# rwickman/ArbitraryStyleTransfer

Hardware: AMD Instinct MI355X
Metric: stylised images/sec at 512x512 bs=8, 1->8 MI355X; encoder MFMA %-of-peak (higher is better)
Workload: dtype f32

## Files before the change

arbitrarystyletransfer_amd/_lib.py:

```python
from __future__ import annotations

import ctypes
import os

import torch

_HERE = os.path.dirname(os.path.abspath(__file__))
LIB_PATH = os.environ.get("AST_HIP_LIB") or os.path.join(_HERE, "libast_hip.so")

_c_float_p = ctypes.c_void_p
_i = ctypes.c_int
_ll = ctypes.c_longlong
_p = ctypes.c_void_p
_f = ctypes.c_float
_d = ctypes.c_double

SIGNATURES = {
    "ast_version": (ctypes.c_char_p, []),
    "ast_loss_acc_floats": (_i, []),
    "ast_conv3x3_packed_numel": (ctypes.c_size_t, [_i, _i]),
    "ast_conv3x3_pack_weights_f32": (_i, [_p, _p, _i, _i, _p]),
    "ast_conv3x3_pack_split_f32": (_i, [_p, _i, _i, _p]),
    "ast_conv3x3_fwd_f32": (_i, [_p, _p, _p, _p, _p, _p, _p, _p, _i, _i, _i, _i, _i, _i, _i, _p]),
    "ast_conv3x3_num_configs": (_i, []),
    "ast_conv3x3_fwd_f32_cfg": (_i, [_i, _p, _p, _i, _p, _p, _p, _p, _p, _p, _p, _i, _i, _i, _i, _i, _i, _i, _p]),
    "ast_channel_stats_f32": (_i, [_p, _p, _p, _ll, _ll, _i, ctypes.c_float, _p]),
    "ast_adain_f32": (_i, [_p, _p, _p, _i, _i, _i, _i, _i, _i, ctypes.c_double, _i, _p]),
    "ast_plane_normalize_f32": (_i, [_p, _p, _p, _p, _ll, _ll, _p]),
    "ast_adain_backward_f32": (_i, [_p, _p, _p, _p, _p, _i, _i, _i, _i, _i, _i, _d, _i, _p]),
    "ast_adain_stats_f32": (_i, [_p, _p, _p, _p, _i, _i, _i, _i, _i, _d, _i, _p]),
    "ast_conv3x3_pack_weights_ex_f32": (_i, [_p, _p, _i, _i, _i, _p, _p]),
    "ast_conv_act_backward_f32": (_i, [_p, _p, _p, _p, _p, _ll, _i, _i, _p]),
    "ast_relu_mask_f32": (_i, [_p, _p, _p, _ll, _p]),
    "ast_grad_pad_f32": (_i, [_p, _p, _p, _ll, _i, _i, _i, _p]),
    "ast_pad_up_adjoint_f32": (_i, [_p, _p, _ll, _i, _i, _i, _i, _p]),
    "ast_conv3x3_dgrad_f32": (_i, [_i, _p, _p, _p, _p, _p, _p, _i, _i, _i, _i, _i, _i, _p]),
    "ast_dgrad_finish_f32": (_i, [_p, _p, _p, _p, _p, _ll, _i, _i, _i, _p]),
    "ast_dgrad_reflect_border_workspace_floats": (_ll, [_i, _i, _i, _i, _i, _i]),
    "ast_dgrad_reflect_border_f32": (_i, [_p, _p, _p, _p, _p, _ll, _i, _i, _i, _i, _i, _i, _p]),
    "ast_conv3x3_wgrad_workspace_floats": (_ll, [_i, _i, _i, _i, _i, _i]),
# ... 167 lines not shown
```

arbitrarystyletransfer_amd/csrc/conv3x3_igemm.hip:

```cpp
#include <hip/hip_runtime.h>
#include <stdint.h>
#include "../../include/ast_hip.h"
#include "x3.h"
#include "cin3.h"

namespace {

typedef float f32x16 __attribute__((ext_vector_type(16)));
typedef float f32x4 __attribute__((ext_vector_type(4)));

constexpr int TW = 32;

struct ConvArgs {
  const float* x;
  const float* x2;
  int nsplit;
  const float* wp;
  const float* bias;
  float* y_pre;
  float* y_act;
  float* y_pool;
  const float* in_mean;
  const float* in_std;
  int N, Cin, Hin, Win, Cout, H, W;
// ... 996 lines not shown
        rec[196] = 0x57a3u;
      }
    }
#endif
  } else {
#if X3_STAGED_EPI
    __syncthreads();
    store_tiles_staged<RM, RN>(a, acc, n, x0, y0, wm * RM, n0, h, l32, lane,
                               reinterpret_cast<float*>(x3_smem) + wm * 32 * RM * 36);
#else
    store_tiles<RM, RN>(a, acc, n, x0, y0, wm * RM, n0, h, l32);
#endif
  }
  if constexpr (!PER) break;
  }
}

__device__ __forceinline__ void x3_lds_barrier() { asm volatile("s_waitcnt lgkmcnt(0)\n\ts_barrier" ::: "memory"); }
__device__ __forceinline__ const float* x3p_uniform(const float* p) {
  const uint64_t v = reinterpret_cast<uint64_t>(p);
  const uint32_t lo = __builtin_amdgcn_readfirstlane((uint32_t)v), hi = __builtin_amdgcn_readfirstlane((uint32_t)(v >> 32));
  return reinterpret_cast<const float*>(((uint64_t)hi << 32) | lo);
}
__device__ __forceinline__ const ConvArgs& x3p_args() {
  auto p = __builtin_amdgcn_kernarg_segment_ptr();
  asm volatile("" : "+s"(p));
  return *(const ConvArgs*)p;
}

template <int WM, int RM, int RN, int UP, int OCC>
// ... 793 lines not shown
  return (int)hipGetLastError();
}

template <int WM, int RM, int RN, int OCC = 1>
int launch_x3p(const ConvArgs& a, hipStream_t s, int up) {
  if (a.in_mean) return AST_E_UNSUPPORTED;
  if ((int64_t)a.Cin * a.Hin * a.Win * 4 >= ((int64_t)1 << 31)) return AST_E_UNSUPPORTED;
  return up == 2 ? launch_x3p_one<WM, RM, RN, 2, OCC>(a, s) : launch_x3p_one<WM, RM, RN, 1, OCC>(a, s);
}

template <int WM, int RM, int RN, int OCC = 1, bool M16 = false, bool PER = false>
int launch_x3(const ConvArgs& a, hipStream_t s, int up) {
  if (a.in_mean) return AST_E_UNSUPPORTED;
  if ((int64_t)a.Cin * a.Hin * a.Win * 4 >= ((int64_t)1 << 31)) return AST_E_UNSUPPORTED;
  return up == 2 ? launch_x3_one<WM, RM, RN, 2, OCC, M16, PER>(a, s) : launch_x3_one<WM, RM, RN, 1, OCC, M16, PER>(a, s);
}

struct CfgEntry {
  int (*fn)(const ConvArgs&, hipStream_t, int);
  int bn;
  int th;
  int rm;
  int max_cout;
};

const CfgEntry kConfigs[] = {
    {launch_cfg<4, 1, 2, 2, 8>, 64, 8, 2, 0},
    {launch_cfg<4, 1, 2, 2, 4>, 64, 8, 2, 0},
    {launch_cfg<2, 2, 4, 2, 4>, 128, 8, 4, 0},
    {launch_cfg<2, 2, 2, 2, 8>, 128, 4, 2, 0},
// ... 82 lines not shown

int ast_conv3x3_pack_weights_f32(const float* w, float* w_packed, int cout, int cin, void* stream) {
  if (!w || !w_packed) return AST_E_NULLPTR;
  if (cout <= 0 || cin <= 0) return AST_E_SHAPE;
  const int cout_pad = round_up(cout, kCoutAlign), cin_pad = round_up(cin, kCinAlign);
  const int64_t total = (int64_t)cin_pad * 9 * cout_pad;
  const int blocks = (int)std::min<int64_t>((total + 255) / 256, 4096);
  hipLaunchKernelGGL(pack_weights_kernel, dim3(blocks), dim3(256), 0, (hipStream_t)stream, w, w_packed, cout, cin,
                     cout_pad, cin_pad);
  const int e = (int)hipGetLastError();
  return e ? e : ast_conv3x3_pack_split_f32(w_packed, cout, cin, stream);
}

int ast_conv3x3_num_configs(void) { return kNumConfigs; }

#if X3_STAMP
int ast_dbg_x3_stamps(void* host, size_t bytes, int clear) {
  const size_t n = std::min(bytes, sizeof(x3_stamp_buf));
  if (clear) {
    void* d = nullptr;
    const hipError_t e = hipGetSymbolAddress(&d, HIP_SYMBOL(x3_stamp_buf));
    return e ? (int)e : (int)hipMemset(d, 0, sizeof(x3_stamp_buf));
  }
  return (int)hipMemcpyFromSymbol(host, HIP_SYMBOL(x3_stamp_buf), n, 0, hipMemcpyDeviceToHost);
}
#endif

int ast_conv3x3_fwd_f32_cfg(int cfg, const float* x, const float* x2, int n2, const float* w_packed,
                            const float* bias, float* y_pre, float* y_act, float* y_pool, const float* in_mean,
                            const float* in_std, int n, int cin, int h_in, int w_in, int cout, int upsample,
// ... 87 lines not shown
```

arbitrarystyletransfer_amd/csrc/torch_ops.cpp:

```cpp
#include <torch/library.h>
#include <ATen/ATen.h>
#include <c10/hip/HIPStream.h>
#include <c10/core/DeviceGuard.h>

#include <tuple>

#include "../../include/ast_hip.h"

namespace {

void* cur_stream(const at::Tensor& t) {
  return (void*)c10::hip::getCurrentHIPStream(t.device().index()).stream();
}

const char* err_name(int code) {
  switch (code) {
    case AST_E_NULLPTR: return "null pointer";
    case AST_E_SHAPE: return "bad shape";
    case AST_E_UNSUPPORTED: return "unsupported configuration";
    default: return "hipError_t";
  }
}

#define AST_CALL(what, expr)                                                                    \
// ... 43 lines not shown
  const c10::DeviceGuard guard(x.device());
  at::Tensor mean = at::empty({x.size(0), x.size(1), 1, 1}, x.options());
  at::Tensor std_ = at::empty_like(mean);
  AST_CALL("channel_stats", ast_channel_stats_f32(x.data_ptr<float>(), mean.data_ptr<float>(), std_.data_ptr<float>(),
                                                  x.size(0) * x.size(1), x.size(2) * x.size(3), unbiased ? 1 : 0,
                                                  (float)eps, cur_stream(x)));
  return {mean, std_};
}

std::tuple<at::Tensor, at::Tensor> channel_stats_meta(const at::Tensor& x, bool, double) {
  TORCH_CHECK(x.dim() == 4, "channel_stats expects NCHW, got ", x.sizes());
  at::Tensor mean = at::empty({x.size(0), x.size(1), 1, 1}, x.options());
  return {mean, at::empty_like(mean)};
}

at::Tensor conv3x3_pack(const at::Tensor& w_) {
  at::Tensor w = dev_f32(w_, "weight");
  TORCH_CHECK(w.dim() == 4 && w.size(2) == 3 && w.size(3) == 3, "conv3x3 weight must be [cout, cin, 3, 3], got ",
              w.sizes());
  const int cout = (int)w.size(0), cin = (int)w.size(1);
  const c10::DeviceGuard guard(w.device());
  at::Tensor out = at::empty({(int64_t)ast_conv3x3_packed_numel(cout, cin)}, w.options());
  AST_CALL("conv3x3_pack", ast_conv3x3_pack_weights_f32(w.data_ptr<float>(), out.data_ptr<float>(), cout, cin,
                                                        cur_stream(w)));
  return out;
}

at::Tensor conv3x3_pack_meta(const at::Tensor& w) {
  TORCH_CHECK(w.dim() == 4 && w.size(2) == 3 && w.size(3) == 3, "conv3x3 weight must be [cout, cin, 3, 3], got ",
              w.sizes());
  return at::empty({(int64_t)ast_conv3x3_packed_numel((int)w.size(0), (int)w.size(1))}, w.options());
}

struct ConvShape {
  int64_t n, cin, h_in, w_in, H, W;
};

ConvShape conv_shape(const at::Tensor& x, const at::Tensor& w_packed, int64_t cout, int64_t upsample,
                     int64_t pad_mode, bool want_pre, bool want_act, bool want_pool) {
  TORCH_CHECK(x.dim() == 4, "x must be NCHW, got ", x.sizes());
  TORCH_CHECK(upsample == 1 || upsample == 2, "upsample must be 1 or 2");
  TORCH_CHECK(pad_mode == 0 || pad_mode == 1, "pad_mode must be 0 (zeros) or 1 (reflect)");
  TORCH_CHECK(want_pre || want_act || want_pool, "conv3x3: no output requested");
  TORCH_CHECK(cout > 0, "cout must be positive");
  ConvShape s{x.size(0), x.size(1), x.size(2), x.size(3), x.size(2) * upsample, x.size(3) * upsample};
  TORCH_CHECK(w_packed.numel() == (int64_t)ast_conv3x3_packed_numel((int)cout, (int)s.cin),
              "packed weight does not match (cout, cin)");
  TORCH_CHECK(!want_pool || (s.H >= 2 && s.W >= 2), "max-pool needs H, W >= 2");
  return s;
}

std::tuple<at::Tensor, at::Tensor, at::Tensor> conv3x3_fwd(
    const at::Tensor& x_, const at::Tensor& w_packed_, const c10::optional<at::Tensor>& bias_, int64_t cout,
    int64_t upsample, int64_t pad_mode, const c10::optional<at::Tensor>& in_mean_,
    const c10::optional<at::Tensor>& in_std_, bool want_pre, bool want_act, bool want_pool, int64_t cfg) {
  at::Tensor x = dev_f32(x_, "x"), w_packed = dev_f32(w_packed_, "w_packed");
  same_device(x, w_packed, "w_packed");
  const ConvShape s = conv_shape(x, w_packed, cout, upsample, pad_mode, want_pre, want_act, want_pool);
  c10::optional<at::Tensor> bias, in_mean, in_std;
  if (bias_) {
    bias = dev_f32(*bias_, "bias");
// ... 1 lines not shown
    TORCH_CHECK(bias->numel() == cout, "bias size mismatch");
  }
  TORCH_CHECK(in_mean_.has_value() == in_std_.has_value(), "in_mean and in_std go together");
  if (in_mean_) {
    in_mean = dev_f32(*in_mean_, "in_mean");
    in_std = dev_f32(*in_std_, "in_std");
    same_device(x, *in_mean, "in_mean");
    same_device(x, *in_std, "in_std");
    TORCH_CHECK(in_mean->numel() == s.cin && in_std->numel() == s.cin, "normalisation stats must have cin entries");
  }
  const c10::DeviceGuard guard(x.device());
  auto mk = [&](bool want, int64_t h, int64_t w) {
    return want ? at::empty({s.n, cout, h, w}, x.options()) : at::empty({0}, x.options());
  };
  at::Tensor pre = mk(want_pre, s.H, s.W), act = mk(want_act, s.H, s.W), pool = mk(want_pool, s.H / 2, s.W / 2);
  AST_CALL("conv3x3", ast_conv3x3_fwd_f32_cfg(
                          (int)cfg, x.data_ptr<float>(), nullptr, 0, w_packed.data_ptr<float>(), fptr(bias),
                          want_pre ? pre.data_ptr<float>() : nullptr, want_act ? act.data_ptr<float>() : nullptr,
                          want_pool ? pool.data_ptr<float>() : nullptr, fptr(in_mean), fptr(in_std), (int)s.n,
                          (int)s.cin, (int)s.h_in, (int)s.w_in, (int)cout, (int)upsample, (int)pad_mode,
                          cur_stream(x)));
  return {pre, act, pool};
}

std::tuple<at::Tensor, at::Tensor, at::Tensor> conv3x3_fwd_meta(
    const at::Tensor& x, const at::Tensor& w_packed, const c10::optional<at::Tensor>&, int64_t cout,
    int64_t upsample, int64_t pad_mode, const c10::optional<at::Tensor>&, const c10::optional<at::Tensor>&,
    bool want_pre, bool want_act, bool want_pool, int64_t) {
  const ConvShape s = conv_shape(x, w_packed, cout, upsample, pad_mode, want_pre, want_act, want_pool);
  auto mk = [&](bool want, int64_t h, int64_t w) {
// ... 13 lines not shown
  AST_CALL("gram", ast_gram_f32(f.data_ptr<float>(), g.data_ptr<float>(), (int)b, (int)c, hw,
                                (float)(1.0 / (double)(c * hw)), ws.data_ptr<float>(), wsf, cur_stream(f)));
  return g;
}

at::Tensor gram_meta(const at::Tensor& f) {
  TORCH_CHECK(f.dim() == 4, "gram_matrix expects [B, C, H, W], got ", f.sizes());
  return at::empty({f.size(0), f.size(1), f.size(1)}, f.options());
}

}

TORCH_LIBRARY(ast_hip, m) {
  m.def("adain(Tensor content_map, Tensor style_map, float alpha=1.0, bool swap_style_stats=True) -> Tensor");
  m.def("channel_stats(Tensor x, bool unbiased=True, float eps=0.0) -> (Tensor, Tensor)");
  m.def("conv3x3_pack(Tensor weight) -> Tensor");
  m.def("conv3x3_fwd(Tensor x, Tensor w_packed, Tensor? bias, int cout, int upsample=1, int pad_mode=0, "
        "Tensor? in_mean=None, Tensor? in_std=None, bool want_pre=False, bool want_act=True, bool want_pool=False, "
        "int cfg=-1) -> (Tensor, Tensor, Tensor)");
  m.def("gram(Tensor feat) -> Tensor");
}

TORCH_LIBRARY_IMPL(ast_hip, CUDA, m) {
  m.impl("adain", &adain);
  m.impl("channel_stats", &channel_stats);
  m.impl("conv3x3_pack", &conv3x3_pack);
  m.impl("conv3x3_fwd", &conv3x3_fwd);
  m.impl("gram", &gram);
}

TORCH_LIBRARY_IMPL(ast_hip, Meta, m) {
// ... 7 lines not shown
```

arbitrarystyletransfer_amd/models.py:

```python
from __future__ import annotations

import torch
import torch.nn as nn
import torch.nn.functional as F

from . import functional as Fn
from . import mbtrain, ops, synth
from .conf import *
from .conf import device
from .losses import *
from .model_util import channel_stats, lab2rgb, rgb2lab

IMNET_MEAN = (0.485, 0.456, 0.406)
IMNET_STD = (0.229, 0.224, 0.225)


class AdaIN(nn.Module):

    def __init__(self, canonical: bool = False):
        super().__init__()
        self.canonical = canonical

    def forward(self, content_map, style_map, alpha: float = 1.0):
        if _compiling():
# ... 74 lines not shown



class _Named:
    @staticmethod
    def name(m: nn.Module, n: str) -> nn.Module:
        m.name = n
        return m


class _PackedConvCache:

    def __init__(self):
        self._cache = {}

    def get(self, conv: nn.Conv2d) -> torch.Tensor:
        w = conv.weight
        key = id(conv)
        stamp = (w.data_ptr(), w._version, w.device, ops.weight_epoch(w))
        hit = self._cache.get(key)
        if hit is not None and hit[0] == stamp:
            return hit[1]
        packed = ops.pack_conv3x3(w.detach())
        self._cache[key] = (stamp, packed)
        return packed


class PretrainedEncoder(nn.Module):

    def __init__(self, content_layers=("conv_1", "conv_3", "conv_5", "conv_9", "conv_13", "relu_15"),
                 weights="live", seed: int = 1):
        super().__init__()
        self._content_layers = set(content_layers)
        norm = _Named.name(Normalization(IMNET_MEAN, IMNET_STD), "norm")
        layers = [norm]
        i, cin = 0, 3
        for v in synth.VGG19_CFG:
            if v == "M":
# ... 116 lines not shown
                layers.append(nn.ReLU())
        super().__init__(*layers)
        self._groups = []
        up = False
        mods = list(self)
        for k, m in enumerate(mods):
            if isinstance(m, nn.Upsample):
                up = True
            elif isinstance(m, nn.Conv2d):
                relu = k + 1 < len(mods) and isinstance(mods[k + 1], nn.ReLU)
                self._groups.append((m, up, relu))
                up = False
        if weights == "live":
            self.load_live_init(seed)
        object.__setattr__(self, "_packed", _PackedConvCache())

    def convs(self):
        return [g[0] for g in self._groups]

    @torch.no_grad()
    def load_live_init(self, seed: int = 2):
        for conv, (w, b) in zip(self.convs(), synth.vgg_decoder_weights(seed)):
            conv.weight.copy_(torch.from_numpy(w))
            conv.bias.copy_(torch.from_numpy(b))

    def forward(self, x):
        if _compiling():
            A = _ops()
            for conv, up, relu in self._groups:
                pre, act, _ = A.conv3x3(x, conv.weight, A.conv3x3_pack(conv.weight.detach()), conv.bias,
                                        2 if up else 1, 1, None, None, not relu, relu, False, None)
                x = act if relu else pre
            return x
        if _needs_grad(x, self):
            g = self._groups
            for k, (conv, up, relu) in enumerate(g):
                x = Fn.DecoderConvFn.apply(x, conv.weight, conv.bias, self._packed.get(conv), 2 if up else 1, relu,
                                           k > 0 and g[k - 1][2], relu and k + 1 < len(g))
            return x
        for conv, up, relu in self._groups:
            pre, act, _ = ops.conv3x3(x, self._packed.get(conv), conv.bias, conv.out_channels,
                                      upsample=2 if up else 1, pad_mode="reflect",
                                      want_pre=not relu, want_act=relu)
            x = act if relu else pre
        return x


class AdaINStyleTransfer(nn.Module):

    def __init__(self, canonical: bool = False, enc_seed: int = 1, dec_seed: int = 2, weights="live"):
        super().__init__()
        self.encoder = PretrainedEncoder(content_layers=["relu_9"], weights=weights, seed=enc_seed)
        self.adain = AdaIN(canonical=canonical)
        self.decoder = VGGDecoder(weights=weights, seed=dec_seed)

    def encode_pair(self, content_img, style_img):
# ... 243 lines not shown
```

arbitrarystyletransfer_amd/ops.py:

```python
from __future__ import annotations

import os

import torch

from ._lib import HipOpError, check, lib, ptr, stream_ptr

PAD_MODES = {"zeros": 0, "reflect": 1}

WEIGHTS_EPOCH = [0]


def bump_weights_epoch(params=None):
    WEIGHTS_EPOCH[0] += 1
    for p in params or ():
        p._ast_epoch = getattr(p, "_ast_epoch", 0) + 1


def weight_epoch(t) -> int:
    return getattr(t, "_ast_epoch", 0)


class LaunchTimer:

# ... 44 lines not shown
def tuned_config(n, cin, h_in, w_in, cout, up, pad_mode, pool, kind="") -> int:
    global _TUNING
    if _TUNING is None:
        import json
        import os
        path = os.environ.get("AST_CONV_TUNING") or os.path.join(
            os.path.dirname(os.path.abspath(__file__)), "conv_tuning.json")
        try:
            with open(path) as f:
                _TUNING = json.load(f)
        except (OSError, ValueError):
            _TUNING = {}
    k = f"{n}x{cin}x{h_in}x{w_in}->{cout} up{up} {pad_mode}{' pool' if pool else ''}{kind}"
    return int(_TUNING.get(k, -1))

def pack_conv3x3(weight: torch.Tensor) -> torch.Tensor:
    w = _dev(weight, "weight")
    if w.dim() != 4 or w.shape[2:] != (3, 3):
        raise HipOpError(f"conv3x3 weight must be [cout, cin, 3, 3], got {tuple(w.shape)}")
    cout, cin = int(w.shape[0]), int(w.shape[1])
    L = lib()
    out = torch.empty(int(L.ast_conv3x3_packed_numel(cout, cin)), device=w.device, dtype=torch.float32)
    check(L.ast_conv3x3_pack_weights_f32(ptr(w), ptr(out), cout, cin, stream_ptr(w.device)), "pack_conv3x3")
    return out


def pack_plan(n: int, w: int, pool: bool):
    if os.environ.get("AST_CONV_PACK", "1") == "0" or n < 2 or w > 64 or (pool and w % 2):
        return 1, 0
    gap = 2 if pool else 1
    base = w / (-(-w // 32) * 32)
    best_u, best_g = base, 1
    for g in range(2, min(n, 8) + 1):
        wp = g * (w + gap) - gap
        u = n * w / (-(-n // g) * (-(-wp // 32) * 32))
        if u > best_u * 1.0001:
            best_u, best_g = u, g
    return (best_g, gap) if best_u >= 1.15 * base else (1, 0)
# ... 2 lines not shown
def conv3x3(x: torch.Tensor, w_packed: torch.Tensor, bias, cout: int, *, upsample: int = 1,
            pad_mode: str = "zeros", in_mean=None, in_std=None,
            want_pre: bool = False, want_act: bool = True, want_pool: bool = False, cfg: int = -1,
            x2: torch.Tensor | None = None, _pack: bool = True, _flops=None):
    x = _dev(x, "x")
    if x.dim() != 4:
        raise HipOpError(f"x must be NCHW, got {tuple(x.shape)}")
    n1, cin, h_in, w_in = (int(s) for s in x.shape)
    n2 = 0
    if x2 is not None:
        x2 = _dev(x2, "x2")
        if x2.dim() != 4 or tuple(x2.shape[1:]) != tuple(x.shape[1:]) or x2.device != x.device:
            raise HipOpError(f"x2 {tuple(x2.shape)} must match x {tuple(x.shape)} in C, H, W")
        n2 = int(x2.shape[0])
    n = n1 + n2
    if w_packed.numel() != int(lib().ast_conv3x3_packed_numel(cout, cin)):
        raise HipOpError("packed weight does not match (cout, cin)")
    if bias is not None:
        bias = _dev(bias, "bias")
        if bias.numel() != cout:
            raise HipOpError("bias size mismatch")
    if (in_mean is None) != (in_std is None):
        raise HipOpError("in_mean and in_std go together")
    if in_mean is not None:
        in_mean, in_std = _dev(in_mean, "in_mean"), _dev(in_std, "in_std")
        if in_mean.numel() != cin or in_std.numel() != cin:
            raise HipOpError("normalisation stats must have cin entries")
    if pad_mode not in PAD_MODES:
        raise HipOpError(f"pad_mode must be one of {list(PAD_MODES)}")
    H, W = h_in * upsample, w_in * upsample
    mk = lambda hh, ww: torch.empty((n, cout, hh, ww), device=x.device, dtype=torch.float32)
    pre = mk(H, W) if want_pre else None
    act = mk(H, W) if want_act else None
    pool = mk(H // 2, W // 2) if want_pool else None
    if pool is not None and (H < 2 or W < 2):
        raise HipOpError("max-pool needs H, W >= 2")
    if pre is None and act is None and pool is None:
        raise HipOpError("conv3x3: no output requested")
    if cfg < 0:
        cfg = tuned_config(n, cin, h_in, w_in, cout, upsample, pad_mode, want_pool)
    G, gap = pack_plan(n, w_in, want_pool) if (_pack and pad_mode == "zeros" and upsample == 1
                                                and in_mean is None) else (1, 0)
    if G > 1:
        L = lib()
        ng, wp = -(-n // G), G * (w_in + gap) - gap
        xp = torch.empty((ng, cin, h_in, wp), device=x.device, dtype=torch.float32)
        check(L.ast_pack_images_f32(ptr(x), n1, ptr(x2), n2, cin, h_in, w_in, G, gap, ptr(xp),
                                    stream_ptr(x.device)), "pack")
        outs = conv3x3(xp, w_packed, bias, cout, want_pre=want_pre, want_act=want_act, want_pool=want_pool,
                       cfg=cfg, _pack=False, _flops=2 * n * H * W * cout * cin * 9)
        res = []
        for t, full, hh, ww in ((outs[0], pre, H, W), (outs[1], act, H, W), (outs[2], pool, H // 2, W // 2)):
            if t is not None:
                sp, wpp = (w_in + gap, wp) if hh == H else ((w_in + gap) // 2, wp // 2)
                check(L.ast_unpack_images_f32(ptr(t), n, cout, hh, ww, G, sp, wpp, ptr(full), stream_ptr(x.device)),
                      "unpack")
            res.append(full if t is not None else None)
        return tuple(res)
    flops = _flops if _flops is not None else 2 * n * H * W * cout * cin * 9
    tag = f"conv3x3 {cin}->{cout} {H}x{W} up{upsample} {pad_mode}"
    code = _timed(tag, flops, x.device, lambda: lib().ast_conv3x3_fwd_f32_cfg(
        cfg, ptr(x), ptr(x2), n2, ptr(w_packed), ptr(bias), ptr(pre), ptr(act), ptr(pool), ptr(in_mean),
        ptr(in_std), n1, cin, h_in, w_in, cout, upsample, PAD_MODES[pad_mode], stream_ptr(x.device)))
    check(code, "conv3x3")
    return pre, act, pool



def channel_stats(x: torch.Tensor, unbiased: bool = True, eps: float = 0.0):
    x = _dev(x, "x")
    if x.dim() != 4:
        raise HipOpError("channel_stats expects NCHW")
    n, c, h, w = x.shape
    mean = torch.empty((n, c, 1, 1), device=x.device, dtype=torch.float32)
    std = torch.empty_like(mean)
# ... 200 lines not shown
```

include/ast_hip.h:

```cpp
#ifndef AST_HIP_H
#define AST_HIP_H

#include <stddef.h>

#ifdef __cplusplus
extern "C" {
#endif

#define AST_OK 0
#define AST_E_NULLPTR (-1)
#define AST_E_SHAPE (-2)
#define AST_E_UNSUPPORTED (-3)

const char* ast_version(void);

#define AST_LOSS_SLOTS 4096
#define AST_LOSS_ACC_FLOATS (2 + AST_LOSS_SLOTS)
int ast_loss_acc_floats(void);


size_t ast_conv3x3_packed_numel(int cout, int cin);

int ast_conv3x3_pack_weights_f32(const float* w, float* w_packed, int cout, int cin, void* stream);

int ast_conv3x3_pack_split_f32(float* w_packed, int cout, int cin, void* stream);

int ast_conv3x3_fwd_f32(const float* x, const float* w_packed, const float* bias,
                        float* y_pre, float* y_act, float* y_pool,
                        const float* in_mean, const float* in_std,
                        int n, int cin, int h_in, int w_in, int cout,
                        int upsample, int pad_mode, void* stream);

int ast_conv3x3_num_configs(void);
int ast_conv3x3_fwd_f32_cfg(int cfg, const float* x, const float* x2, int n2,
                            const float* w_packed, const float* bias,
                            float* y_pre, float* y_act, float* y_pool,
                            const float* in_mean, const float* in_std,
                            int n, int cin, int h_in, int w_in, int cout,
                            int upsample, int pad_mode, void* stream);


int ast_channel_stats_f32(const float* x, float* mean, float* std, long long planes, long long hw,
                          int unbiased, float eps, void* stream);

int ast_adain_f32(const float* content, const float* style, float* out,
                  int n, int c, int hc, int wc, int hs, int ws,
                  double alpha, int swap_style_stats, void* stream);

int ast_adain_stats_f32(const float* content, const float* style_mean, const float* style_std,
                        float* out, int n, int c, int hc, int wc, int style_stride_n, double alpha,
                        int swap_style_stats, void* stream);

int ast_adain_backward_f32(const float* content, const float* style, const float* grad_out,
                           float* d_content, float* d_style, int n, int c, int hc, int wc,
// ... 310 lines not shown
```

Measured before the change: 607.1.

## Add phase-decomposed upsample-2x conv kernel with collapsed 2x2 weights

Adds a dedicated kernel for nearest-upsample-by-2 followed by reflect-padded 3x3 conv. It splits the output into four sub-pixel phases and pre-sums the 3x3 weights into 2x2 taps per phase, so the conv reads the low-resolution input directly and does about 16/36 of the MACs. Weights are packed once into a bf16 three-way split tail appended to the packed buffer, and the decoder uses this path by default on the inference path. This adds a new pack step and cache key. Reflect handling at borders must match the original upsample-then-pad semantics, and summing the weights in double and rounding once changes the rounding slightly.

```diff
diff --git a/arbitrarystyletransfer_amd/_lib.py b/arbitrarystyletransfer_amd/_lib.py
--- a/arbitrarystyletransfer_amd/_lib.py
+++ b/arbitrarystyletransfer_amd/_lib.py
@@ -24,6 +24,9 @@
     "ast_conv3x3_fwd_f32": (_i, [_p, _p, _p, _p, _p, _p, _p, _p, _i, _i, _i, _i, _i, _i, _i, _p]),
     "ast_conv3x3_num_configs": (_i, []),
     "ast_conv3x3_fwd_f32_cfg": (_i, [_i, _p, _p, _i, _p, _p, _p, _p, _p, _p, _p, _i, _i, _i, _i, _i, _i, _i, _p]),
+    "ast_conv3x3_up2c_numel": (ctypes.c_size_t, [_i, _i]),
+    "ast_conv3x3_pack_up2c_f32": (_i, [_p, _p, _i, _i, _p]),
+    "ast_conv3x3_up2c_fwd_f32": (_i, [_p, _p, _i, _p, _p, _p, _p, _i, _i, _i, _i, _i, _i, _i, _p]),
     "ast_channel_stats_f32": (_i, [_p, _p, _p, _ll, _ll, _i, ctypes.c_float, _p]),
     "ast_adain_f32": (_i, [_p, _p, _p, _i, _i, _i, _i, _i, _i, ctypes.c_double, _i, _p]),
     "ast_plane_normalize_f32": (_i, [_p, _p, _p, _p, _ll, _ll, _p]),
diff --git a/arbitrarystyletransfer_amd/csrc/conv3x3_igemm.hip b/arbitrarystyletransfer_amd/csrc/conv3x3_igemm.hip
--- a/arbitrarystyletransfer_amd/csrc/conv3x3_igemm.hip
+++ b/arbitrarystyletransfer_amd/csrc/conv3x3_igemm.hip
@@ -1034,6 +1034,261 @@
   }
   if constexpr (!PER) break;
   }
+}
+
+constexpr int kUp2cTaps = 16;
+constexpr int kUp2cBN = 32;
+
+__host__ __device__ constexpr int64_t up2c_numel(int cin, int cout) {
+  return (int64_t)((cin + kX3K - 1) / kX3K * kX3K) * kUp2cTaps * ((cout + 63) / 64 * 64) * 3 / 2;
+}
+
+__host__ __device__ constexpr int up2c_tap(int t) { return (int)((0xFEBAD7C693825410ull >> (4 * t)) & 15); }
+__host__ __device__ constexpr int up2c_pos(int c) { return ((c >> 3) + ((c >> 1) & 1)) * 3 + ((c >> 2) & 1) + (c & 1); }
+
+__global__ void pack_up2c_kernel(const float* __restrict__ wp, bf16* __restrict__ ws, int cin_pad8, int cin16,
+                                 int cout_pad) {
+  const int64_t total = (int64_t)cin16 * kUp2cTaps * cout_pad;
+  for (int64_t idx = (int64_t)blockIdx.x * blockDim.x + threadIdx.x; idx < total;
+       idx += (int64_t)gridDim.x * blockDim.x) {
+    const int co = (int)(idx % cout_pad);
+    const int64_t rt = idx / cout_pad;
+    const int c = (int)(rt % kUp2cTaps);
+    const int ci = (int)(rt / kUp2cTaps);
+    const int py = c >> 3, px = (c >> 2) & 1, ta = (c >> 1) & 1, tb = c & 1;
+    const int ky0 = ta == 0 ? 0 : (py == 0 ? 1 : 2), ky1 = ta == 0 ? (py == 0 ? 0 : 1) : 2;
+    const int kx0 = tb == 0 ? 0 : (px == 0 ? 1 : 2), kx1 = tb == 0 ? (px == 0 ? 0 : 1) : 2;
+    double s = 0.0;
+    if (ci < cin_pad8)
+      for (int ky = ky0; ky <= ky1; ++ky)
+        for (int kx = kx0; kx <= kx1; ++kx) s += (double)wp[((int64_t)ci * 9 + ky * 3 + kx) * cout_pad + co];
+    bf16 t[3];
+    split3((float)s, t[0], t[1], t[2]);
+    const int kc = ci / kX3K, hh = (ci >> 3) & 1, e = ci & 7;
+#pragma unroll
+    for (int p = 0; p < 3; ++p)
+      ws[((((int64_t)(kc * 3 + p) * kUp2cTaps + c) * 2 + hh) * cout_pad + co) * 8 + e] = t[p];
+  }
+}
+
+template <int WM>
+struct Up2cCfg {
+  using X = X3Cfg<WM, 4, 1, 2>;
+  static_assert(X::BN == kUp2cBN && X::TH == 4 * WM, "");
+  static constexpr int B_ROWS = 3 * kUp2cTaps * 2;
+  static constexpr int B_PLANE = kUp2cTaps * 2 * kUp2cBN;
+  static constexpr int B_UNITS = B_ROWS * kUp2cBN;
+  static constexpr int LDS_TILES = (X::A_UNITS + 2 * B_UNITS) * 16;
+  static constexpr int LDS_BYTES = LDS_TILES > X::LDS_EPI ? LDS_TILES : X::LDS_EPI;
+};
+
+template <int WM>
+__global__ __launch_bounds__(WM * 64, 1) void conv3x3_up2c_kernel(ConvArgs a, const u32x4* __restrict__ wc) {
+  using U = Up2cCfg<WM>;
+  using C = typename U::X;
+  constexpr int NT = C::NT, TH = C::TH, BN = kUp2cBN, SR = C::SR, SC = C::SC, A_PLANE = C::A_PLANE;
+  constexpr int HS = C::HS, A_ITEMS = C::A_ITEMS, A_T = C::A_T;
+  constexpr int B_UNITS = U::B_UNITS, B_PLANE = U::B_PLANE;
+  extern __shared__ __attribute__((aligned(16))) u32x4 x3_smem[];
+  u32x4* As = x3_smem;
+  u32x4* Bs = x3_smem + C::A_UNITS;
+
+  const int tid = threadIdx.x, wm = tid >> 6, lane = tid & 63;
+  const int ntl = a.tiles_x * a.tiles_y * a.N, ngr = (a.Cout + BN - 1) / BN;
+  int t, grp;
+  if (!decode_block(blockIdx.x, ntl, ngr, t, grp)) return;
+  const int tx = t % a.tiles_x;
+  t /= a.tiles_x;
+  const int ty = t % a.tiles_y;
+  const int n = t / a.tiles_y;
+  const int x0 = tx * TW, y0 = ty * TH;
+  const int sx0 = x0 / 2, sy0 = y0 / 2 - 1;
+  const int n0 = grp * BN;
+  const int Hin = a.Hin, Win = a.Win, plane_in = Hin * Win;
+  const float* __restrict__ xin =
+      n < a.nsplit ? a.x + (int64_t)n * a.Cin * plane_in : a.x2 + (int64_t)(n - a.nsplit) * a.Cin * plane_in;
+  const int nch = (a.Cin + kX3K - 1) / kX3K;
+  const int64_t chunk_units = (int64_t)U::B_ROWS * a.cout_pad;
+
+  unsigned g_off[A_T], g_pix[A_T];
+  int g_lds[A_T], g_h[A_T];
+#pragma unroll
+  for (int i = 0; i < A_T; ++i) {
+    const int e = min(tid + i * NT, A_ITEMS - 1);
+    const int c = e % SC, rest = e / SC, r = rest % SR, hh = rest / SR;
+    const int sy = src_index<2>(sy0 + r, Hin, 1), sx = src_index<2>(sx0 - 1 + c, Win, 1);
+    g_pix[i] = (unsigned)(sy * Win + sx);
+    g_off[i] = 4u * (unsigned)(8 * hh * plane_in) + 4u * g_pix[i];
+    g_lds[i] = hh * HS + r * SC + c;
+    g_h[i] = hh;
+  }
+  const int plane_b = 4 * plane_in;
+  float ra[A_T][8];
+  bf16x8 pv[A_T][3];
+#define UP2C_LOAD_A(KC, I0, I1)                                                                         \
+  {                                                                                                     \
+    const int ci0 = (KC) * kX3K;                                                                        \
+    if (ci0 + kX3K <= a.Cin) {                                                                          \
+      const __amdgpu_buffer_rsrc_t xr = __builtin_amdgcn_make_buffer_rsrc(                              \
+          const_cast<float*>(xin + (int64_t)ci0 * plane_in), 0, kX3K * plane_b, 0x00020000);           \
+      _Pragma("unroll") for (int j = 0; j < 8; ++j)                                                     \
+        _Pragma("unroll") for (int i = (I0); i < (I1); ++i)                                             \
+          ra[i][j] = __builtin_bit_cast(float, __builtin_amdgcn_raw_buffer_load_b32(xr, (int)g_off[i], j * plane_b, 0)); \
+    } else {                                                                                            \
+      _Pragma("unroll") for (int i = (I0); i < (I1); ++i)                                               \
+        _Pragma("unroll") for (int j = 0; j < 8; ++j)                                                   \
+          ra[i][j] = xin[(int64_t)min(ci0 + 8 * g_h[i] + j, a.Cin - 1) * plane_in + g_pix[i]];          \
+    }                                                                                                   \
+  }
+  static_assert(B_UNITS % (64 * WM) == 0, "whole 1-KiB pieces, the same count per wave");
+#define UP2C_DMA(KC)                                                                                    \
+  _Pragma("unroll") for (int i = 0; i < B_UNITS / 64 / WM; ++i) {                                       \
+    const int piece = wm + i * WM;                                                                      \
+    const int u = piece * 64 + lane, row = u / BN, j = u - row * BN;                                    \
+    const u32x4* src = wc + (int64_t)(KC) * chunk_units + (int64_t)row * a.cout_pad + n0 + j;           \
+    __builtin_amdgcn_global_load_lds((const void*)src,                                                  \
+                                     (__attribute__((address_space(3))) void*)(Bs + ((KC) & 1) * B_UNITS + piece * 64), \
+                                     16, 0, 0);                                                         \
+  }
+#define UP2C_SPLIT_A(KC)                                                                                \
+  _Pragma("unroll") for (int i = 0; i < A_T; ++i) {                                                     \
+    if ((KC) * kX3K + kX3K > a.Cin) {                         \
+      const int cn = a.Cin - (KC) * kX3K - 8 * g_h[i];                                                  \
+      _Pragma("unroll") for (int j = 0; j < 8; ++j) ra[i][j] = j < cn ? ra[i][j] : 0.f;                  \
+    }                                                                                                   \
+    ast_x3::split8(ra[i], pv[i][0], pv[i][1], pv[i][2]);                                                \
+  }
+#define UP2C_WRITE_A                                                                                    \
+  _Pragma("unroll") for (int i = 0; i < A_T; ++i)                                                       \
+    if (tid + i * NT < A_ITEMS)                                                                         \
+      _Pragma("unroll") for (int p = 0; p < 3; ++p)                                                     \
+        As[p * A_PLANE + g_lds[i]] = __builtin_bit_cast(u32x4, pv[i][p]);
+
+  typedef float f32x4v __attribute__((ext_vector_type(4)));
+  f32x4v acc[2][2][2][2];
+#pragma unroll
+  for (int r = 0; r < 2; ++r)
+#pragma unroll
+    for (int p = 0; p < 4; ++p)
+#pragma unroll
+      for (int q = 0; q < 2; ++q) acc[r][p >> 1][p & 1][q] = f32x4v{0.f, 0.f, 0.f, 0.f};
+
+  const int l16 = lane & 15, g16 = lane >> 4, hh16 = g16 & 1;
+  const int apl1 = (g16 < 2 ? 0 : 1) * A_PLANE, apl2 = (g16 < 2 ? 0 : 2) * A_PLANE;
+  const int arow = hh16 * HS + (2 * wm) * SC + l16;
+
+  UP2C_DMA(0);
+  UP2C_LOAD_A(0, 0, A_T);
+  UP2C_SPLIT_A(0);
+  UP2C_WRITE_A;
+  asm volatile("s_waitcnt vmcnt(0)" ::: "memory");
+  __syncthreads();
+  static_assert(A_T < kUp2cTaps - 1, "one gather item per step, then the slab DMA");
+  for (int kc = 0; kc < nch; ++kc) {
+    __builtin_amdgcn_sched_barrier(0);
+    bf16x8 gb[2][3][2];
+    bf16x8 fa[2][2][2];
+    const u32x4* __restrict__ bs = Bs + (kc & 1) * B_UNITS;
+    const u32x4* __restrict__ bp1 = bs;
+    const u32x4* __restrict__ bp2 = bs + (g16 < 2 ? B_PLANE : 0);
+    const u32x4* __restrict__ bp3 = bs + (g16 < 2 ? 2 * B_PLANE : B_PLANE);
+#define UP2C_READ_B(BUF, TAP)                                                                           \
+    _Pragma("unroll") for (int q = 0; q < 2; ++q) {                                                     \
+      const int bi = ((TAP) * 2 + hh16) * BN + q * 16 + l16;                                            \
+      gb[BUF][0][q] = __builtin_bit_cast(bf16x8, bp1[bi]);                                              \
+      gb[BUF][1][q] = __builtin_bit_cast(bf16x8, bp2[bi]);                                              \
+      gb[BUF][2][q] = __builtin_bit_cast(bf16x8, bp3[bi]);                                              \
+    }
+#define UP2C_READ_A(POS)                                                                                \
+    _Pragma("unroll") for (int r = 0; r < 2; ++r) {                                                     \
+      const int ai = arow + (r + (POS) / 3) * SC + (POS) % 3;                                           \
+      fa[(POS) & 1][r][0] = __builtin_bit_cast(bf16x8, As[apl1 + ai]);                                  \
+      fa[(POS) & 1][r][1] = __builtin_bit_cast(bf16x8, As[apl2 + ai]);                                  \
+    }
+    UP2C_READ_B(0, up2c_tap(0));
+    UP2C_READ_A(0);
+#pragma unroll
+    for (int st = 0; st < kUp2cTaps; ++st) {
+      const int c = up2c_tap(st), py = c >> 3, px = (c >> 2) & 1, pos = up2c_pos(c), ab = pos & 1, bb = st & 1;
+      if (st < A_T && kc + 1 < nch) {
+        __builtin_amdgcn_sched_barrier(0);
+        UP2C_LOAD_A(kc + 1, st, st + 1)
+        __builtin_amdgcn_sched_barrier(0);
+      }
+      if (st == A_T && kc + 1 < nch) {
+        __builtin_amdgcn_sched_barrier(0);
+        UP2C_DMA(kc + 1);
+        __builtin_amdgcn_sched_barrier(0);
+      }
+      int nrd = 0;
+      if (st + 1 < kUp2cTaps) {
+        UP2C_READ_B(bb ^ 1, up2c_tap(st + 1));
+        nrd = 6;
+        if (up2c_pos(up2c_tap(st + 1)) != pos) {
+          UP2C_READ_A(up2c_pos(up2c_tap(st + 1)));
+          nrd += 4;
+        }
+      }
+#pragma unroll
+      for (int r = 0; r < 2; ++r)
+#pragma unroll
+        for (int q = 0; q < 2; ++q)
+          acc[r][py][px][q] = __builtin_amdgcn_mfma_f32_16x16x32_bf16(fa[ab][r][0], gb[bb][2][q], acc[r][py][px][q], 0, 0, 0);
+#pragma unroll
+      for (int r = 0; r < 2; ++r)
+#pragma unroll
+        for (int q = 0; q < 2; ++q)
+          acc[r][py][px][q] = __builtin_amdgcn_mfma_f32_16x16x32_bf16(fa[ab][r][1], gb[bb][1][q], acc[r][py][px][q], 0, 0, 0);
+#pragma unroll
+      for (int r = 0; r < 2; ++r)
+#pragma unroll
+        for (int q = 0; q < 2; ++q)
+          acc[r][py][px][q] = __builtin_amdgcn_mfma_f32_16x16x32_bf16(fa[ab][r][0], gb[bb][0][q], acc[r][py][px][q], 0, 0, 0);
+#pragma unroll
+      for (int r = 0; r < nrd; ++r) {
+        __builtin_amdgcn_sched_group_barrier(0x100, 1, 0);
+        __builtin_amdgcn_sched_group_barrier(0x008, 1, 0);
+      }
+      if (nrd == 10) __builtin_amdgcn_sched_group_barrier(0x008, 2, 0);
+      else if (nrd == 6) __builtin_amdgcn_sched_group_barrier(0x008, 6, 0);
+      else __builtin_amdgcn_sched_group_barrier(0x008, 12, 0);
+      __builtin_amdgcn_sched_barrier(0);
+    }
+#undef UP2C_READ_A
+#undef UP2C_READ_B
+    __builtin_amdgcn_sched_barrier(0);
+    if (kc + 1 < nch) {
+      UP2C_SPLIT_A(kc + 1);
+      asm volatile("s_waitcnt vmcnt(0)" ::: "memory");
+      __syncthreads();
+      UP2C_WRITE_A;
+      __syncthreads();
+    }
+  }
+#undef UP2C_LOAD_A
+#undef UP2C_DMA
+#undef UP2C_SPLIT_A
+#undef UP2C_WRITE_A
+
+  __syncthreads();
+  float* region = reinterpret_cast<float*>(x3_smem) + wm * 32 * 4 * 36;
+#pragma unroll
+  for (int q = 0; q < 2; ++q) {
+    const int co = n0 + 16 * q + l16;
+    const float bv = (co < a.Cout && a.bias) ? a.bias[co] : 0.f;
+#pragma unroll
+    for (int r = 0; r < 2; ++r)
+#pragma unroll
+      for (int py = 0; py < 2; ++py) {
+        const f32x4v v0 = acc[r][py][0][q], v1 = acc[r][py][1][q];
+        float* dst = region + ((16 * q + l16) * 4 + 2 * r + py) * 36 + 8 * g16;
+        *reinterpret_cast<float4*>(dst) = make_float4(v0[0] + bv, v1[0] + bv, v0[1] + bv, v1[1] + bv);
+        *reinterpret_cast<float4*>(dst + 4) = make_float4(v0[2] + bv, v1[2] + bv, v0[3] + bv, v1[3] + bv);
+      }
+  }
+  __builtin_amdgcn_s_waitcnt(0xc07f);
+  __builtin_amdgcn_wave_barrier();
+  store_region<4>(a, region, n, x0, y0, 4 * wm, n0, lane);
 }
 
 __device__ __forceinline__ void x3_lds_barrier() { asm volatile("s_waitcnt lgkmcnt(0)\n\ts_barrier" ::: "memory"); }
@@ -1857,6 +2112,26 @@
   if (a.in_mean) return AST_E_UNSUPPORTED;
   if ((int64_t)a.Cin * a.Hin * a.Win * 4 >= ((int64_t)1 << 31)) return AST_E_UNSUPPORTED;
   return up == 2 ? launch_x3_one<WM, RM, RN, 2, OCC, M16, PER>(a, s) : launch_x3_one<WM, RM, RN, 1, OCC, M16, PER>(a, s);
+}
+
+int launch_up2c(const ConvArgs& a0, const float* w_up2c, hipStream_t s) {
+  using U = Up2cCfg<8>;
+  ConvArgs a = a0;
+  a.tiles_x = cdiv(a.W, TW);
+  a.tiles_y = cdiv(a.H, U::X::TH);
+  const int64_t ntiles = (int64_t)a.tiles_x * a.tiles_y * a.N;
+  const int64_t nblk = (ntiles + 7) / 8 * 8 * cdiv(a.Cout, kUp2cBN);
+  if (nblk >= 0x7fffffff) return AST_E_SHAPE;
+  auto kern = conv3x3_up2c_kernel<8>;
+  constexpr int lds = U::LDS_BYTES;
+  static_assert(lds <= 160 * 1024, "LDS per CU");
+  static bool attr_set = false;
+  if (!attr_set) {
+    (void)hipFuncSetAttribute((const void*)kern, hipFuncAttributeMaxDynamicSharedMemorySize, lds);
+    attr_set = true;
+  }
+  hipLaunchKernelGGL(kern, dim3((unsigned)nblk), dim3(U::X::NT), lds, s, a, reinterpret_cast<const u32x4*>(w_up2c));
+  return (int)hipGetLastError();
 }
 
 struct CfgEntry {
@@ -1969,6 +2244,43 @@
 
 int ast_conv3x3_num_configs(void) { return kNumConfigs; }
 
+size_t ast_conv3x3_up2c_numel(int cout, int cin) {
+  if (cout <= 0 || cin <= 0) return 0;
+  return (size_t)up2c_numel(cin, cout);
+}
+
+int ast_conv3x3_pack_up2c_f32(const float* w_packed, float* w_up2c, int cout, int cin, void* stream) {
+  if (!w_packed || !w_up2c) return AST_E_NULLPTR;
+  if (cout <= 0 || cin <= 0) return AST_E_SHAPE;
+  const int cout_pad = round_up(cout, kCoutAlign);
+  const int64_t total = (int64_t)round_up(cin, kX3K) * kUp2cTaps * cout_pad;
+  const int blocks = (int)std::min<int64_t>((total + 255) / 256, 4096);
+  hipLaunchKernelGGL(pack_up2c_kernel, dim3(blocks), dim3(256), 0, (hipStream_t)stream, w_packed,
+                     reinterpret_cast<bf16*>(w_up2c), round_up(cin, kCinAlign), round_up(cin, kX3K), cout_pad);
+  return (int)hipGetLastError();
+}
+
+int ast_conv3x3_up2c_fwd_f32(const float* x, const float* x2, int n2, const float* w_up2c, const float* bias,
+                             float* y_pre, float* y_act, int n, int cin, int h_in, int w_in, int cout, int upsample,
+                             int pad_mode, void* stream) {
+  if (!x || !w_up2c) return AST_E_NULLPTR;
+  if (n2 < 0 || (n2 > 0 && !x2)) return AST_E_NULLPTR;
+  if (!y_pre && !y_act) return AST_E_NULLPTR;
+  if (n <= 0 || cin <= 0 || h_in <= 0 || w_in <= 0 || cout <= 0) return AST_E_SHAPE;
+  if (upsample != 2 || pad_mode != 1 || cin < kX3K) return AST_E_UNSUPPORTED;
+  if ((reinterpret_cast<uintptr_t>(w_up2c) & 15) != 0) return AST_E_UNSUPPORTED;
+  if ((int64_t)cin * h_in * w_in * 4 >= ((int64_t)1 << 31)) return AST_E_UNSUPPORTED;
+  if ((int64_t)round_up(cin, kX3K) * kUp2cTaps * round_up(cout, kCoutAlign) >= ((int64_t)1 << 31)) return AST_E_SHAPE;
+  ConvArgs a{};
+  a.x = x; a.x2 = x2; a.nsplit = n; a.bias = bias;
+  a.y_pre = y_pre; a.y_act = y_act;
+  a.N = n + n2; a.Cin = cin; a.Hin = h_in; a.Win = w_in; a.Cout = cout; a.H = 2 * h_in; a.W = 2 * w_in;
+  a.cin_pad = round_up(cin, kCinAlign);
+  a.cout_pad = round_up(cout, kCoutAlign);
+  a.reflect = 1;
+  return launch_up2c(a, w_up2c, (hipStream_t)stream);
+}
+
 #if X3_STAMP
 int ast_dbg_x3_stamps(void* host, size_t bytes, int clear) {
   const size_t n = std::min(bytes, sizeof(x3_stamp_buf));
diff --git a/arbitrarystyletransfer_amd/csrc/torch_ops.cpp b/arbitrarystyletransfer_amd/csrc/torch_ops.cpp
--- a/arbitrarystyletransfer_amd/csrc/torch_ops.cpp
+++ b/arbitrarystyletransfer_amd/csrc/torch_ops.cpp
@@ -81,22 +81,28 @@
   return {mean, at::empty_like(mean)};
 }
 
-at::Tensor conv3x3_pack(const at::Tensor& w_) {
+at::Tensor conv3x3_pack(const at::Tensor& w_, bool up2c) {
   at::Tensor w = dev_f32(w_, "weight");
   TORCH_CHECK(w.dim() == 4 && w.size(2) == 3 && w.size(3) == 3, "conv3x3 weight must be [cout, cin, 3, 3], got ",
               w.sizes());
   const int cout = (int)w.size(0), cin = (int)w.size(1);
   const c10::DeviceGuard guard(w.device());
-  at::Tensor out = at::empty({(int64_t)ast_conv3x3_packed_numel(cout, cin)}, w.options());
+  const int64_t base = (int64_t)ast_conv3x3_packed_numel(cout, cin);
+  at::Tensor out = at::empty({base + (up2c ? (int64_t)ast_conv3x3_up2c_numel(cout, cin) : 0)}, w.options());
   AST_CALL("conv3x3_pack", ast_conv3x3_pack_weights_f32(w.data_ptr<float>(), out.data_ptr<float>(), cout, cin,
                                                         cur_stream(w)));
+  if (up2c)
+    AST_CALL("conv3x3_pack up2c", ast_conv3x3_pack_up2c_f32(out.data_ptr<float>(), out.data_ptr<float>() + base, cout,
+                                                            cin, cur_stream(w)));
   return out;
 }
 
-at::Tensor conv3x3_pack_meta(const at::Tensor& w) {
+at::Tensor conv3x3_pack_meta(const at::Tensor& w, bool up2c) {
   TORCH_CHECK(w.dim() == 4 && w.size(2) == 3 && w.size(3) == 3, "conv3x3 weight must be [cout, cin, 3, 3], got ",
               w.sizes());
-  return at::empty({(int64_t)ast_conv3x3_packed_numel((int)w.size(0), (int)w.size(1))}, w.options());
+  const int cout = (int)w.size(0), cin = (int)w.size(1);
+  return at::empty({(int64_t)ast_conv3x3_packed_numel(cout, cin) +
+                    (up2c ? (int64_t)ast_conv3x3_up2c_numel(cout, cin) : 0)}, w.options());
 }
 
 struct ConvShape {
@@ -111,7 +117,9 @@
   TORCH_CHECK(want_pre || want_act || want_pool, "conv3x3: no output requested");
   TORCH_CHECK(cout > 0, "cout must be positive");
   ConvShape s{x.size(0), x.size(1), x.size(2), x.size(3), x.size(2) * upsample, x.size(3) * upsample};
-  TORCH_CHECK(w_packed.numel() == (int64_t)ast_conv3x3_packed_numel((int)cout, (int)s.cin),
+  const int64_t base = (int64_t)ast_conv3x3_packed_numel((int)cout, (int)s.cin);
+  TORCH_CHECK(w_packed.numel() == base ||
+                  w_packed.numel() == base + (int64_t)ast_conv3x3_up2c_numel((int)cout, (int)s.cin),
               "packed weight does not match (cout, cin)");
   TORCH_CHECK(!want_pool || (s.H >= 2 && s.W >= 2), "max-pool needs H, W >= 2");
   return s;
@@ -143,6 +151,15 @@
     return want ? at::empty({s.n, cout, h, w}, x.options()) : at::empty({0}, x.options());
   };
   at::Tensor pre = mk(want_pre, s.H, s.W), act = mk(want_act, s.H, s.W), pool = mk(want_pool, s.H / 2, s.W / 2);
+  const int64_t base = (int64_t)ast_conv3x3_packed_numel((int)cout, (int)s.cin);
+  if (w_packed.numel() > base && upsample == 2 && pad_mode == 1 && !want_pool && s.cin >= 16 && !in_mean && cfg < 0) {
+    AST_CALL("conv3x3 up2c", ast_conv3x3_up2c_fwd_f32(
+                                 x.data_ptr<float>(), nullptr, 0, w_packed.data_ptr<float>() + base, fptr(bias),
+                                 want_pre ? pre.data_ptr<float>() : nullptr, want_act ? act.data_ptr<float>() : nullptr,
+                                 (int)s.n, (int)s.cin, (int)s.h_in, (int)s.w_in, (int)cout, (int)upsample,
+                                 (int)pad_mode, cur_stream(x)));
+    return {pre, act, pool};
+  }
   AST_CALL("conv3x3", ast_conv3x3_fwd_f32_cfg(
                           (int)cfg, x.data_ptr<float>(), nullptr, 0, w_packed.data_ptr<float>(), fptr(bias),
                           want_pre ? pre.data_ptr<float>() : nullptr, want_act ? act.data_ptr<float>() : nullptr,
@@ -186,7 +203,7 @@
 TORCH_LIBRARY(ast_hip, m) {
   m.def("adain(Tensor content_map, Tensor style_map, float alpha=1.0, bool swap_style_stats=True) -> Tensor");
   m.def("channel_stats(Tensor x, bool unbiased=True, float eps=0.0) -> (Tensor, Tensor)");
-  m.def("conv3x3_pack(Tensor weight) -> Tensor");
+  m.def("conv3x3_pack(Tensor weight, bool up2c=False) -> Tensor");
   m.def("conv3x3_fwd(Tensor x, Tensor w_packed, Tensor? bias, int cout, int upsample=1, int pad_mode=0, "
         "Tensor? in_mean=None, Tensor? in_std=None, bool want_pre=False, bool want_act=True, bool want_pool=False, "
         "int cfg=-1) -> (Tensor, Tensor, Tensor)");
diff --git a/arbitrarystyletransfer_amd/models.py b/arbitrarystyletransfer_amd/models.py
--- a/arbitrarystyletransfer_amd/models.py
+++ b/arbitrarystyletransfer_amd/models.py
@@ -112,14 +112,14 @@
     def __init__(self):
         self._cache = {}
 
-    def get(self, conv: nn.Conv2d) -> torch.Tensor:
+    def get(self, conv: nn.Conv2d, up2c: bool = False) -> torch.Tensor:
         w = conv.weight
-        key = id(conv)
+        key = (id(conv), up2c)
         stamp = (w.data_ptr(), w._version, w.device, ops.weight_epoch(w))
         hit = self._cache.get(key)
         if hit is not None and hit[0] == stamp:
             return hit[1]
-        packed = ops.pack_conv3x3(w.detach())
+        packed = ops.pack_conv3x3(w.detach(), up2c=up2c)
         self._cache[key] = (stamp, packed)
         return packed
 
@@ -266,6 +266,7 @@
         if weights == "live":
             self.load_live_init(seed)
         object.__setattr__(self, "_packed", _PackedConvCache())
+        object.__setattr__(self, "_up2c", ops.up2c_enabled())
 
     def convs(self):
         return [g[0] for g in self._groups]
@@ -279,9 +280,10 @@
     def forward(self, x):
         if _compiling():
             A = _ops()
+            tail = self._up2c and not _needs_grad(x, self)
             for conv, up, relu in self._groups:
-                pre, act, _ = A.conv3x3(x, conv.weight, A.conv3x3_pack(conv.weight.detach()), conv.bias,
-                                        2 if up else 1, 1, None, None, not relu, relu, False, None)
+                pre, act, _ = A.conv3x3(x, conv.weight, A.conv3x3_pack(conv.weight.detach(), up and tail),
+                                        conv.bias, 2 if up else 1, 1, None, None, not relu, relu, False, None)
                 x = act if relu else pre
             return x
         if _needs_grad(x, self):
@@ -291,7 +293,7 @@
                                            k > 0 and g[k - 1][2], relu and k + 1 < len(g))
             return x
         for conv, up, relu in self._groups:
-            pre, act, _ = ops.conv3x3(x, self._packed.get(conv), conv.bias, conv.out_channels,
+            pre, act, _ = ops.conv3x3(x, self._packed.get(conv, up and self._up2c), conv.bias, conv.out_channels,
                                       upsample=2 if up else 1, pad_mode="reflect",
                                       want_pre=not relu, want_act=relu)
             x = act if relu else pre
diff --git a/arbitrarystyletransfer_amd/ops.py b/arbitrarystyletransfer_amd/ops.py
--- a/arbitrarystyletransfer_amd/ops.py
+++ b/arbitrarystyletransfer_amd/ops.py
@@ -82,14 +82,30 @@
     k = f"{n}x{cin}x{h_in}x{w_in}->{cout} up{up} {pad_mode}{' pool' if pool else ''}{kind}"
     return int(_TUNING.get(k, -1))
 
-def pack_conv3x3(weight: torch.Tensor) -> torch.Tensor:
+
+_UP2C = None
+
+
+def up2c_enabled() -> bool:
+    global _UP2C
+    if _UP2C is None:
+        _UP2C = os.environ.get("AST_CONV_UP2C", "1") != "0"
+    return _UP2C
+
+
+def pack_conv3x3(weight: torch.Tensor, up2c: bool = False) -> torch.Tensor:
     w = _dev(weight, "weight")
     if w.dim() != 4 or w.shape[2:] != (3, 3):
         raise HipOpError(f"conv3x3 weight must be [cout, cin, 3, 3], got {tuple(w.shape)}")
     cout, cin = int(w.shape[0]), int(w.shape[1])
     L = lib()
-    out = torch.empty(int(L.ast_conv3x3_packed_numel(cout, cin)), device=w.device, dtype=torch.float32)
+    base = int(L.ast_conv3x3_packed_numel(cout, cin))
+    tail = int(L.ast_conv3x3_up2c_numel(cout, cin)) if up2c else 0
+    out = torch.empty(base + tail, device=w.device, dtype=torch.float32)
     check(L.ast_conv3x3_pack_weights_f32(ptr(w), ptr(out), cout, cin, stream_ptr(w.device)), "pack_conv3x3")
+    if up2c:
+        check(L.ast_conv3x3_pack_up2c_f32(ptr(out), ptr(out[base:]), cout, cin, stream_ptr(w.device)),
+              "pack_conv3x3 up2c")
     return out
 
 
@@ -122,7 +138,9 @@
             raise HipOpError(f"x2 {tuple(x2.shape)} must match x {tuple(x.shape)} in C, H, W")
         n2 = int(x2.shape[0])
     n = n1 + n2
-    if w_packed.numel() != int(lib().ast_conv3x3_packed_numel(cout, cin)):
+    base = int(lib().ast_conv3x3_packed_numel(cout, cin))
+    has_tail = w_packed.numel() == base + int(lib().ast_conv3x3_up2c_numel(cout, cin))
+    if w_packed.numel() != base and not has_tail:
         raise HipOpError("packed weight does not match (cout, cin)")
     if bias is not None:
         bias = _dev(bias, "bias")
@@ -145,6 +163,8 @@
         raise HipOpError("max-pool needs H, W >= 2")
     if pre is None and act is None and pool is None:
         raise HipOpError("conv3x3: no output requested")
+    up2c = (has_tail and upsample == 2 and pad_mode == "reflect" and not want_pool and cin >= 16
+            and in_mean is None and cfg < 0)
     if cfg < 0:
         cfg = tuned_config(n, cin, h_in, w_in, cout, upsample, pad_mode, want_pool)
     G, gap = pack_plan(n, w_in, want_pool) if (_pack and pad_mode == "zeros" and upsample == 1
@@ -167,6 +187,12 @@
         return tuple(res)
     flops = _flops if _flops is not None else 2 * n * H * W * cout * cin * 9
     tag = f"conv3x3 {cin}->{cout} {H}x{W} up{upsample} {pad_mode}"
+    if up2c:
+        code = _timed(tag, flops, x.device, lambda: lib().ast_conv3x3_up2c_fwd_f32(
+            ptr(x), ptr(x2), n2, ptr(w_packed[base:]), ptr(bias), ptr(pre), ptr(act), n1, cin, h_in, w_in, cout,
+            upsample, PAD_MODES[pad_mode], stream_ptr(x.device)))
+        check(code, "conv3x3 up2c")
+        return pre, act, pool
     code = _timed(tag, flops, x.device, lambda: lib().ast_conv3x3_fwd_f32_cfg(
         cfg, ptr(x), ptr(x2), n2, ptr(w_packed), ptr(bias), ptr(pre), ptr(act), ptr(pool), ptr(in_mean),
         ptr(in_std), n1, cin, h_in, w_in, cout, upsample, PAD_MODES[pad_mode], stream_ptr(x.device)))
diff --git a/include/ast_hip.h b/include/ast_hip.h
--- a/include/ast_hip.h
+++ b/include/ast_hip.h
@@ -38,6 +38,13 @@
                             const float* in_mean, const float* in_std,
                             int n, int cin, int h_in, int w_in, int cout,
                             int upsample, int pad_mode, void* stream);
+
+size_t ast_conv3x3_up2c_numel(int cout, int cin);
+int ast_conv3x3_pack_up2c_f32(const float* w_packed, float* w_up2c, int cout, int cin, void* stream);
+int ast_conv3x3_up2c_fwd_f32(const float* x, const float* x2, int n2, const float* w_up2c,
+                             const float* bias, float* y_pre, float* y_act,
+                             int n, int cin, int h_in, int w_in, int cout,
+                             int upsample, int pad_mode, void* stream);
 
 
 int ast_channel_stats_f32(const float* x, float* mean, float* std, long long planes, long long hw,
```

After: 640.9 (median of 6 runs). 1.06x the previous value.
